# ZhuoyangLiu2005/MLA

Measured on AMD Instinct MI355X. Metric: training samples/sec + step-time, MLA-Llama2-7B bf16, higher is better.
Workload: dtype bf16; 1 GPU; BASELINE.json configs[1]: MLA-Llama2-7B SFT, use_pointcloud+use_contrastive, 672x672(+mask) image + 1024 points + 32 text tokens, per-GPU batch 8 x 4 diffusion repeats = 32 x 548 tokens; model=mla-llama2-7b, global_batch=8, seq_len=548, parallelism=single-gpu, activation_save_level=1, optimizer=fused AdamW + grad clip inside the timed region

## Files before the change

### mla_amd/csrc/gemm256.hip

```cpp
#include "common.h"

#include "gemm_args.h"

#include "gemm256_kloop_clobbers.inc"
#ifndef MLA_GEMM_PLAIN_STORES
#define MLA_ST16(ADDR, VAL) __builtin_nontemporal_store((u32x4_t)(VAL), (u32x4_t*)(ADDR))
#define MLA_LD16(ADDR) __builtin_nontemporal_load((const u32x4_t*)(ADDR))
#else
#define MLA_ST16(ADDR, VAL) (*(u32x4_t*)(ADDR) = (VAL))
#define MLA_LD16(ADDR) (*(const u32x4_t*)(ADDR))
#endif

namespace {

constexpr int SLOT = 16384;
constexpr int SA0 = 0, SB0 = SLOT, SB1 = 2 * SLOT, SA1 = 3 * SLOT, BUF = 4 * SLOT;

__device__ __forceinline__ int hsw(int kr) { return (kr & 3) | (((kr >> 3) & 1) << 2); }
__device__ __forceinline__ int xcd_remap(int bid, int nwg) {
  const int q = nwg >> 3, r = nwg & 7;
  const int xcd = bid & 7, idx = bid >> 3;
  return (xcd < r ? xcd * (q + 1) : r * (q + 1) + (xcd - r) * q) + idx;
}

template <int MODE, bool IS_A>
__device__ __forceinline__ const bf16_t* stage_src(const bf16_t* g, int ld, int base, int lim, int h, int instr, int lane) {
  const int p = instr * 64 + lane;
  if (MODE == 0) {
    const int rp = p >> 3, cp = p & 7;
    const int c = cp ^ (rp & 7);
    int gi = base + h * 128 + rp;
    gi = gi < lim ? gi : lim - 1;
    return g + (size_t)gi * ld + c * 8;
  } else {
    const int kr = p >> 4, cp = p & 15;
    const int c = cp ^ (hsw(kr) << 1);
    const int ip = c * 8;
    int gi = base + h * 128 + ip;
    gi = (gi + 8 <= lim) ? gi : 0;
    return g + (size_t)kr * ld + gi;
  }
}

#ifndef MLA_GROUP_M
#define MLA_GROUP_M 4
#endif
#ifndef MLA_GEMM256_UNTRACKED
#define MLA_GEMM256_UNTRACKED 0
#endif
template <int AMODE, int BMODE, int EPI = 0, bool ASM = false>
__global__ __launch_bounds__(512, 2) void gemm256_kernel(GemmArgs p) {
  const bool LGKM_BEFORE = false;
  const int GROUP_M = MLA_GROUP_M;
#ifdef MLA_GEMM256_ABLATION
  const bool NO_READ = (p.debug & 4) != 0, NO_STAGE = (p.debug & 8) != 0, NO_BAR2 = (p.debug & 16) != 0, NO_BAR1 = (p.debug & 32) != 0;
  const int dbg = p.debug;
#else
  constexpr bool NO_READ = false, NO_STAGE = false, NO_BAR2 = false, NO_BAR1 = false;
  constexpr int dbg = 0;
#endif
  extern __shared__ __attribute__((aligned(16))) char smem[];
  const int tid = threadIdx.x, lane = tid & 63;
  const int wave = __builtin_amdgcn_readfirstlane(tid >> 6);
  const int wr = wave >> 2, wc = wave & 3;
  const int li = lane & 15, lg = lane >> 4;

  const int num_m = (p.M + 255) / 256, num_n = (p.N + 255) / 256;
  int pid, kt0 = 0, nt = p.K / 64;
  float* part = nullptr;
  if (p.sk_split <= 1) {
    pid = xcd_remap(blockIdx.x, gridDim.x);
  } else if ((int)blockIdx.x < p.sk_full) {
    pid = xcd_remap(blockIdx.x, p.sk_full);
  } else {
    const int u = blockIdx.x - p.sk_full;
    const int slice = u % p.sk_split;
    pid = p.sk_full + u / p.sk_split;
    if ((nt & 1) == 0) {
      const int np = nt >> 1;
      kt0 = 2 * (int)((long long)slice * np / p.sk_split);
      nt = 2 * (int)((long long)(slice + 1) * np / p.sk_split) - kt0;
    } else {
    kt0 = (int)((long long)slice * nt / p.sk_split);
    nt = (int)((long long)(slice + 1) * nt / p.sk_split) - kt0;
    }
    part = p.sk_ws + (size_t)u * 65536;
  }
#ifdef MLA_EXPERIMENTAL_KERNELS
  if (EPI != 0 && p.stagger_mode && (int)blockIdx.x < 256) {
    const bool late = p.stagger_mode == 1 ? (blockIdx.x & 1) : ((blockIdx.x >> 3) & 1);
    if (late) {
      const unsigned long long t0 = wall_clock64();
      while ((long long)(wall_clock64() - t0) < (long long)p.stagger_ticks) __builtin_amdgcn_s_sleep(64);
    }
  }
#endif
  const int in_group = GROUP_M * num_n;
  const int group_id = pid / in_group;
  const int first_m = group_id * GROUP_M;
  const int gsz = (num_m - first_m) < GROUP_M ? (num_m - first_m) : GROUP_M;
  const int pid_m = first_m + (pid % in_group) % gsz;
  const int pid_n = (pid % in_group) / gsz;
  const int m0 = pid_m * 256, n0 = pid_n * 256;

  f32x4_t acc[8][4];
  if constexpr (ASM) {
    static_assert(AMODE == 0 && BMODE == 0, "the assembly loop takes k-contiguous operands");
    const unsigned c0 = ((unsigned)lg ^ ((unsigned)li & 7u)) << 4;
    const unsigned vA0 = (unsigned)((wr * 64 + li) * 128) + c0, vB0 = 32768u + (unsigned)((wc * 32 + li) * 128) + c0;
    const unsigned lchunk = ((unsigned)lane & 7u) ^ (((unsigned)lane >> 3) & 7u);
    const int rt0 = wave * 32 + (lane >> 3);
    const int lastA = (p.M - 1 - m0) < 255 ? (p.M - 1 - m0) : 255;
    int lastB = (p.N - 1 - n0) < 255 ? (p.N - 1 - n0) : 255, bshift = 0;
    const bf16_t* pB = p.B + (size_t)n0 * p.ldb + (size_t)kt0 * 64;
    if (EPI == 1) {
      pB = p.B + (size_t)pid_n * 128 * p.ldb;
      bshift = wave >= 4 ? p.sf_I - 128 : 0;
      lastB = 255;
    }
    const unsigned oA0 = (unsigned)rt0 * (unsigned)p.lda * 2u + lchunk * 16u;
    const unsigned oB0 = (unsigned)(rt0 + bshift) * (unsigned)p.ldb * 2u + lchunk * 16u;
    const unsigned oAmax = (unsigned)lastA * (unsigned)p.lda * 2u + lchunk * 16u;
    const unsigned oBmax = (unsigned)(lastB + bshift) * (unsigned)p.ldb * 2u + lchunk * 16u;
    const int sA8 = p.lda * 16, sB8 = p.ldb * 16;
    const bf16_t* pA = p.A + (size_t)m0 * p.lda + (size_t)kt0 * 64;
    const int kmax = nt * 128 - 128, nit = nt >> 1, ldsw = wave * 4096;
    const bool img_bf16 = !part && !p.out_fp32 && p.R == nullptr && p.bias == nullptr;
    const bool rowscale = img_bf16 && p.rs_rstd != nullptr;
    if (rowscale && tid < 256) {
      const int mr = (m0 + tid) < p.M ? (m0 + tid) : (p.M - 1);
      float r;
      if (p.rs_ss) {
        const float* sp = p.rs_ss + (size_t)mr * p.rs_parts;
        float t = 0.f;
        for (int j = 0; j < p.rs_parts; ++j) t += sp[j];
        r = 1.0f / sqrtf(t / (float)p.K + p.rs_eps);
        if (pid_n == 0 && m0 + tid < p.M) p.rs_rstd[mr] = r;
      } else {
        r = p.rs_rstd[mr];
      }
      *(float*)(smem + 2 * BUF + tid * 4) = r;
    }
    const int emode = img_bf16 ? (rowscale ? 2 : 0) : 1;
    const float alpha = part ? 1.f : p.alpha;
    const unsigned vImg = img_bf16 ? (unsigned)((wr * 64 + li) * 512) + ((((unsigned)(wc * 4 + (lg >> 1))) ^ (unsigned)li) << 4) + (unsigned)(lg & 1) * 8u
                                   : (unsigned)((wr * 64 + li) * 1024) + ((((unsigned)(wc * 8 + lg)) ^ (unsigned)li) << 4);
#if defined(__HIP_DEVICE_COMPILE__)
    asm volatile(
#include "gemm256_kloop.inc"
        : : [pA] "s"(pA), [pB] "s"(pB), [kmax] "v"(kmax), [nit] "v"(nit), [ldsw] "s"(ldsw), [sA8] "s"(sA8), [sB8] "s"(sB8),
            [emode] "v"(emode), [alpha] "v"(alpha), [vA0] "v"(vA0), [vB0] "v"(vB0), [oA0] "v"(oA0), [oB0] "v"(oB0), [oAmax] "v"(oAmax),
            [oBmax] "v"(oBmax), [vImg] "v"(vImg)
        : "memory", "scc", "vcc", "s40", "s41", "s42", "s43", "s44", "s45", "s46", "s47", "s48", "s49", "s50", "s51", "s52", "s53", G256K_CLOBBERS);
#endif
    if constexpr (EPI == 0) if (part) {
#pragma unroll
      for (int hf = 0; hf < 2; ++hf) {
        if (hf) {
          __syncthreads();
#if defined(__HIP_DEVICE_COMPILE__)
          asm volatile(
#include "gemm256_kloop_half1.inc"
              : : [alpha] "v"(alpha), [vImg] "v"(vImg) : "memory", "v0", "v1", "v2", "v3", "v4", "v5", "v6", "v7", "v8", "v9", "v10", "v11",
                "v12", "v13", "v14", "v15", "v16", "v17", "v18", "v19");
#endif
        }
        __syncthreads();
#pragma unroll
        for (int it = 0; it < 16; ++it) {
          const int row = wave * 16 + it;
          *(f32x4_t*)(part + (hf * 128 + row) * 256 + lane * 4) = *(const f32x4_t*)(smem + row * 1024 + ((lane ^ (row & 63)) << 4));
        }
      }
      return;
    }
  } else {
  const size_t stepA = (dbg & 64) ? 0 : (dbg & 2) ? 64 : (AMODE == 0 ? 64 : (size_t)64 * p.lda);
  const size_t stepB = (dbg & 64) ? 0 : (dbg & 2) ? 64 : (BMODE == 0 ? 64 : (size_t)64 * p.ldb);
  const bf16_t* pA0[2]; const bf16_t* pA1[2]; const bf16_t* pB0[2]; const bf16_t* pB1[2];
#pragma unroll
  for (int it = 0; it < 2; ++it) {
    if (dbg & 2) {
      pA0[it] = stage_src<0, true>(p.A, 4096, 0, 4096, 0, wave * 2 + it, lane);
      pA1[it] = stage_src<0, true>(p.A, 4096, 0, 4096, 1, wave * 2 + it, lane);
      pB0[it] = stage_src<0, false>(p.B, 4096, 0, 4096, 0, wave * 2 + it, lane);
      pB1[it] = stage_src<0, false>(p.B, 4096, 0, 4096, 1, wave * 2 + it, lane);
      continue;
    }
    pA0[it] = stage_src<AMODE, true>(p.A, p.lda, m0, p.M, 0, wave * 2 + it, lane);
    pA1[it] = stage_src<AMODE, true>(p.A, p.lda, m0, p.M, 1, wave * 2 + it, lane);
    if (EPI == 1) {
      pB0[it] = stage_src<BMODE, false>(p.B, p.ldb, pid_n * 128, p.sf_I, 0, wave * 2 + it, lane);
      pB1[it] = stage_src<BMODE, false>(p.B, p.ldb, p.sf_I + pid_n * 128 - 128, 2 * p.sf_I, 1, wave * 2 + it, lane);
      continue;
    }
    pB0[it] = stage_src<BMODE, false>(p.B, p.ldb, n0, p.N, 0, wave * 2 + it, lane);
    pB1[it] = stage_src<BMODE, false>(p.B, p.ldb, n0, p.N, 1, wave * 2 + it, lane);
  }
  if (kt0) {
#pragma unroll
    for (int it = 0; it < 2; ++it) {
      pA0[it] += (size_t)kt0 * stepA; pA1[it] += (size_t)kt0 * stepA;
      pB0[it] += (size_t)kt0 * stepB; pB1[it] += (size_t)kt0 * stepB;
    }
  }
  int tA0 = 0, tA1 = 0, tB0 = 0, tB1 = 0;
  constexpr bool UNTRACKED = (AMODE != 0 || BMODE != 0) || MLA_GEMM256_UNTRACKED;

#define STAGE(PTR, TCNT, STEP, SLOTOFF)                                                           \
  do {                                                                                            \
    const size_t back__ = (TCNT < nt) ? 0 : (size_t)TCNT * (STEP);  \
    char* dst__ = smem + (TCNT & 1) * BUF + (SLOTOFF) + wave * 2048;                              \
    if (!NO_STAGE || TCNT < 2) {  \
      if (UNTRACKED) {                                                                            \
        glds16_untracked(PTR[0] - back__, dst__);                                                 \
        glds16_untracked(PTR[1] - back__, dst__ + 1024);                                          \
      } else {                                                                                    \
        glds16(PTR[0] - back__, dst__);                                                           \
        glds16(PTR[1] - back__, dst__ + 1024);                                                    \
      }                                                                                           \
    }                                                                                             \
    PTR[0] += (STEP); PTR[1] += (STEP); ++TCNT;                                                   \
  } while (0)

  int offA[4], offB[2];
  if (AMODE == 0) {
    offA[0] = (wr * 64 + li) * 128 + ((lg ^ (li & 7)) * 16);
    offA[1] = offA[2] = offA[3] = 0;
  } else {
    const int h = ((li >> 2) & 3) | ((lg & 1) << 2);
#pragma unroll
    for (int rb = 0; rb < 4; ++rb)
      offA[rb] = ((lg * 8 + (li >> 2)) * 16 + ((wr * 8 + rb * 2 + ((li & 3) >> 1)) ^ (h << 1))) * 16 + (li & 1) * 8;
  }
  if (BMODE == 0) {
    offB[0] = (wc * 32 + li) * 128 + ((lg ^ (li & 7)) * 16);
    offB[1] = 0;
  } else {
    const int h = ((li >> 2) & 3) | ((lg & 1) << 2);
#pragma unroll
    for (int cb = 0; cb < 2; ++cb)
      offB[cb] = ((lg * 8 + (li >> 2)) * 16 + ((wc * 4 + cb * 2 + ((li & 3) >> 1)) ^ (h << 1))) * 16 + (li & 1) * 8;
  }

  auto ldA = [&](const char* slot, int rb, int ks) -> bf16x8_t {
    if (AMODE == 0) {
      return *(const bf16x8_t*)(slot + ((offA[0] + rb * 2048) ^ (ks * 64)));
    } else {
      if (dbg & 1) return *(const bf16x8_t*)(slot + (((wr * 64 + li) * 128 + ((lg ^ (li & 7)) * 16) + rb * 2048) ^ (ks * 64)));
      union { bf16x8_t v; short4_t h2[2]; } u;
      u.h2[0] = lds_tr16_b64(slot + offA[rb] + ks * 8192);
      u.h2[1] = lds_tr16_b64(slot + offA[rb] + ks * 8192 + 1024);
      return u.v;
    }
  };
  auto ldB = [&](const char* slot, int cb, int ks) -> bf16x8_t {
    if (BMODE == 0) {
      return *(const bf16x8_t*)(slot + ((offB[0] + cb * 2048) ^ (ks * 64)));
    } else {
      if (dbg & 1) return *(const bf16x8_t*)(slot + (((wc * 32 + li) * 128 + ((lg ^ (li & 7)) * 16) + cb * 2048) ^ (ks * 64)));
      union { bf16x8_t v; short4_t h2[2]; } u;
      u.h2[0] = lds_tr16_b64(slot + offB[cb] + ks * 8192);
      u.h2[1] = lds_tr16_b64(slot + offB[cb] + ks * 8192 + 1024);
      return u.v;
    }
  };

#pragma unroll
  for (int a = 0; a < 8; ++a)
#pragma unroll
    for (int b = 0; b < 4; ++b) acc[a][b] = f32x4_t{0.f, 0.f, 0.f, 0.f};

  bf16x8_t fa[4][2], fb0[2][2], fb1[2][2];
  bool rd_on = true;

#define READ_A(SLOTP)                                              \
  if (rd_on) _Pragma("unroll") for (int rb = 0; rb < 4; ++rb) {    \
    fa[rb][0] = ldA(SLOTP, rb, 0); fa[rb][1] = ldA(SLOTP, rb, 1);  \
  }
#define READ_B(DST, SLOTP)                                          \
  if (rd_on) _Pragma("unroll") for (int cb = 0; cb < 2; ++cb) {     \
    DST[cb][0] = ldB(SLOTP, cb, 0); DST[cb][1] = ldB(SLOTP, cb, 1); \
  }
#define SEG_END()                                                  \
  __builtin_amdgcn_sched_barrier(0);                               \
  if (LGKM_BEFORE) asm volatile("s_waitcnt vmcnt(8) lgkmcnt(0)" ::: "memory"); \
  else asm volatile("s_waitcnt vmcnt(10)" ::: "memory");           \
  if (!NO_BAR1) __builtin_amdgcn_s_barrier();                      \
  asm volatile("s_waitcnt lgkmcnt(0)" ::: "memory");               \
  __builtin_amdgcn_sched_barrier(0);
#define MMA(QI, QJ, FB)                                                                                          \
  __builtin_amdgcn_s_setprio(1);                                                                                 \
  _Pragma("unroll") for (int ks = 0; ks < 2; ++ks)                                                               \
  _Pragma("unroll") for (int rb = 0; rb < 4; ++rb)                                                               \
  _Pragma("unroll") for (int cb = 0; cb < 2; ++cb)                                                               \
    acc[QI * 4 + rb][QJ * 2 + cb] =                                                                              \
        __builtin_amdgcn_mfma_f32_16x16x32_bf16(FB[cb][ks], fa[rb][ks], acc[QI * 4 + rb][QJ * 2 + cb], 0, 0, 0); \
  __builtin_amdgcn_s_setprio(0);                                                                                 \
  __builtin_amdgcn_sched_barrier(0);                                                                             \
  asm volatile("" ::: "memory");                                                                                 \
  if (!NO_BAR2) __builtin_amdgcn_s_barrier();                                                                    \
  asm volatile("" ::: "memory");

  STAGE(pB0, tB0, stepB, SB0);
  STAGE(pA0, tA0, stepA, SA0);
  STAGE(pB1, tB1, stepB, SB1);
  STAGE(pA1, tA1, stepA, SA1);
  STAGE(pB0, tB0, stepB, SB0);
  STAGE(pA0, tA0, stepA, SA0);
  STAGE(pB1, tB1, stepB, SB1);
  asm volatile("s_waitcnt vmcnt(10)" ::: "memory");
  __builtin_amdgcn_s_barrier();
  READ_B(fb0, smem + SB0)
  if (wr == 1) __builtin_amdgcn_s_barrier();

#define TILE_BODY(X, Y, T_)                                          \
  {                                                                  \
    const char* buf = smem + ((T_) & 1) * BUF;                       \
    const char* nbuf = smem + (((T_) + 1) & 1) * BUF;                \
    if (NO_READ) rd_on = (T_) < 2;                                   \
    STAGE(pA1, tA1, stepA, SA1);                       \
    READ_A(buf + SA0)                                                \
    SEG_END()                                                        \
    MMA(0, 0, X)                                                     \
    STAGE(pB0, tB0, stepB, SB0);                       \
    READ_B(Y, buf + SB1)                                             \
    SEG_END()                                                        \
    MMA(0, 1, Y)                                                     \
    STAGE(pA0, tA0, stepA, SA0);                       \
    READ_A(buf + SA1)                                                \
    SEG_END()                                                        \
    MMA(1, 1, Y)                                                     \
    STAGE(pB1, tB1, stepB, SB1);                       \
    READ_B(Y, nbuf + SB0)                                            \
    SEG_END()                                                        \
    MMA(1, 0, X)                                                     \
  }
  int t = 0;
  for (; t + 1 < nt; t += 2) {
    TILE_BODY(fb0, fb1, t)
    TILE_BODY(fb1, fb0, t + 1)
  }
  if (t < nt) TILE_BODY(fb0, fb1, t)
#undef TILE_BODY
  if (wr == 0) __builtin_amdgcn_s_barrier();
  asm volatile("s_waitcnt vmcnt(0)" ::: "memory");
  }

  if constexpr (!ASM) if (part) {
#pragma unroll
    for (int ri = 0; ri < 8; ++ri) {
      const int ml = (ri >> 2) * 128 + wr * 64 + (ri & 3) * 16 + li;
#pragma unroll
      for (int ci = 0; ci < 4; ++ci) {
        const int nl = (ci >> 1) * 128 + wc * 32 + (ci & 1) * 16 + lg * 4;
        *(f32x4_t*)(part + ml * 256 + nl) = acc[ri][ci];
      }
    }
    return;
  }
  const bool vec_ok = ((p.ldc & 3) == 0) && (p.R == nullptr || (p.ldr & 3) == 0);
  const bool fast = (p.N & 7) == 0 && (p.ldc & 7) == 0 && (((uintptr_t)p.C) & 15) == 0 &&
                    (p.R == nullptr || ((p.ldr & 7) == 0 && (((uintptr_t)p.R) & 15) == 0)) &&
                    (p.bias == nullptr || (((uintptr_t)p.bias) & 15) == 0);
  if (fast) {
    __syncthreads();
    if (!p.out_fp32 && p.R == nullptr && p.bias == nullptr) {
      if constexpr (!ASM) {
      if (p.rs_rstd) {
        if (tid < 256) {
          const int mr = (m0 + tid) < p.M ? (m0 + tid) : (p.M - 1);
          float r;
          if (p.rs_ss) {
            const float* sp = p.rs_ss + (size_t)mr * p.rs_parts;
            float t = 0.f;
            for (int j = 0; j < p.rs_parts; ++j) t += sp[j];
            r = 1.0f / sqrtf(t / (float)p.K + p.rs_eps);
            if (pid_n == 0 && m0 + tid < p.M) p.rs_rstd[mr] = r;
          } else {
            r = p.rs_rstd[mr];
          }
          *(float*)(smem + 2 * BUF + tid * 4) = r;
        }
        __syncthreads();
      }
#pragma unroll
      for (int ri = 0; ri < 8; ++ri) {
        const int ml = (ri >> 2) * 128 + wr * 64 + (ri & 3) * 16 + li;
        const float rsc = p.rs_rstd ? *(const float*)(smem + 2 * BUF + ml * 4) : p.alpha;
#pragma unroll
        for (int ci = 0; ci < 4; ++ci) {
          const int nl = (ci >> 1) * 128 + wc * 32 + (ci & 1) * 16 + lg * 4;
          u32x2_t o;
          o[0] = pack2bf(acc[ri][ci][0] * rsc, acc[ri][ci][1] * rsc);
          o[1] = pack2bf(acc[ri][ci][2] * rsc, acc[ri][ci][3] * rsc);
          *(u32x2_t*)(smem + ml * 512 + ((((nl >> 3) ^ (ml & 31))) << 4) + ((nl >> 2) & 1) * 8) = o;
        }
      }
      }
      __syncthreads();
      if (EPI == 1) {
        const int I = p.sf_I, cbase = pid_n * 128;
        const size_t ld2 = (size_t)2 * I;
        for (int s4 = 0; s4 < 4; ++s4) {
          char* scrA = smem + s4 * 64 * 512;
          u32x4_t pa[2];
#pragma unroll
          for (int k4 = 0; k4 < 4; ++k4) {
            const int idx = tid + 512 * k4;
            const int rl = idx >> 5, ch = idx & 31;
            const int row = s4 * 64 + rl, m = m0 + row;
            if (p.C && m < p.M)
              MLA_ST16((bf16_t*)p.C + (size_t)m * ld2 + (ch < 16 ? cbase + ch * 8 : I + cbase + (ch - 16) * 8), *(const u32x4_t*)(smem + row * 512 + ((ch ^ (row & 31)) << 4)));
          }
#pragma unroll
          for (int k2 = 0; k2 < 2; ++k2) {
            const int idx = tid + 512 * k2;
            const int rl = idx >> 4, c = idx & 15;
            const int row = s4 * 64 + rl, m = m0 + row;
            float gv[8], uv[8], o[8];
            unpack8(*(const u32x4_t*)(smem + row * 512 + ((c ^ (row & 31)) << 4)), gv);
            unpack8(*(const u32x4_t*)(smem + row * 512 + (((16 + c) ^ (row & 31)) << 4)), uv);
#pragma unroll
            for (int j = 0; j < 8; ++j) o[j] = swiglu_fwd_elem(gv[j], uv[j]);
            pa[k2] = pack8(o);
            if (p.sf_act && m < p.M) MLA_ST16(p.sf_act + (size_t)m * I + cbase + c * 8, pa[k2]);
          }
          if (p.sf_actT == nullptr) continue;
          __syncthreads();
#pragma unroll
          for (int k2 = 0; k2 < 2; ++k2) {
            const int idx = tid + 512 * k2;
            const int rl = idx >> 4, c = idx & 15;
            const int slot2 = (rl ^ (2 * c)) * 2;
#pragma unroll
            for (int j = 0; j < 4; ++j) {
              const int c0 = (c * 8 + 2 * j) * 128 + slot2;
              *(unsigned short*)(scrA + c0) = (unsigned short)(pa[k2][j] & 0xffffu);
              *(unsigned short*)(scrA + c0 + 128) = (unsigned short)(pa[k2][j] >> 16);
            }
          }
          __syncthreads();
#pragma unroll
          for (int k2 = 0; k2 < 2; ++k2) {
            const int idx = tid + 512 * k2;
            const int col = idx >> 3, rc = idx & 7;
            const int chc = col >> 3, b = chc & 3;
            const int m = m0 + s4 * 64 + rc * 8;
            if (m < p.M) {
              u32x4_t w = *(const u32x4_t*)(scrA + col * 128 + ((rc ^ (chc >> 2)) << 4));
              if (b & 1) w = u32x4_t{w[1], w[0], w[3], w[2]};
              if (b & 2) w = u32x4_t{w[2], w[3], w[0], w[1]};
              MLA_ST16(p.sf_actT + (size_t)(cbase + col) * p.sf_ldt + m, w);
            }
          }
        }
        return;
      }
      if (EPI == 2) {
        const int I = p.sw_I;
        char* scrB = smem + 2 * BUF;
        const size_t ld2 = (size_t)2 * I;
        u32x4_t gq[4], uq[4];
        auto fetch_gu = [&](int strip, u32x4_t* g4, u32x4_t* u4) {
#pragma unroll
          for (int k4 = 0; k4 < 4; ++k4) {
            const int idx = tid + 512 * k4;
            const int m = m0 + strip * 64 + (idx >> 5), n = n0 + (idx & 31) * 8;
            g4[k4] = u32x4_t{0u, 0u, 0u, 0u};
            u4[k4] = g4[k4];
            if (m < p.M && n < p.N) {
              g4[k4] = MLA_LD16(p.sw_gu + (size_t)m * ld2 + n);
              u4[k4] = MLA_LD16(p.sw_gu + (size_t)m * ld2 + I + n);
            }
          }
        };
        if constexpr (ASM) fetch_gu(0, gq, uq);
        for (int s4 = 0; s4 < 4; ++s4) {
          char* scrA = smem + s4 * 64 * 512;
          u32x4_t pg[4], pu[4];
          u32x4_t gn[4], un[4];
          if constexpr (ASM) if (s4 < 3) fetch_gu(s4 + 1, gn, un);
#pragma unroll
          for (int k4 = 0; k4 < 4; ++k4) {
            const int idx = tid + 512 * k4;
            const int rl = idx >> 5, ch = idx & 31;
            const int row = s4 * 64 + rl;
            const int m = m0 + row, n = n0 + ch * 8;
            pg[k4] = u32x4_t{0u, 0u, 0u, 0u};
            pu[k4] = pg[k4];
            if (m < p.M && n < p.N) {
              float dv[8], gv[8], uv[8], dg[8], du[8];
              unpack8(*(const u32x4_t*)(smem + row * 512 + ((ch ^ (row & 31)) << 4)), dv);
              if constexpr (ASM) {
                unpack8(gq[k4], gv);
                unpack8(uq[k4], uv);
              } else {
              unpack8(*(const u32x4_t*)(p.sw_gu + (size_t)m * ld2 + n), gv);
              unpack8(*(const u32x4_t*)(p.sw_gu + (size_t)m * ld2 + I + n), uv);
              }
#pragma unroll
              for (int j = 0; j < 8; ++j) swiglu_bwd_elem(dv[j], gv[j], uv[j], dg[j], du[j]);
              pg[k4] = pack8(dg);
              pu[k4] = pack8(du);
              MLA_ST16(p.sw_dgu + (size_t)m * ld2 + n, pg[k4]);
              MLA_ST16(p.sw_dgu + (size_t)m * ld2 + I + n, pu[k4]);
            }
          }
          __syncthreads();
#pragma unroll
          for (int k4 = 0; k4 < 4; ++k4) {
            const int idx = tid + 512 * k4;
            const int rl = idx >> 5, ch = idx & 31;
            const int slot2 = (rl ^ (2 * ch)) * 2;
#pragma unroll
            for (int j = 0; j < 4; ++j) {
              const int c0 = (ch * 8 + 2 * j) * 128 + slot2;
              *(unsigned short*)(scrA + c0) = (unsigned short)(pg[k4][j] & 0xffffu);
              *(unsigned short*)(scrA + c0 + 128) = (unsigned short)(pg[k4][j] >> 16);
              *(unsigned short*)(scrB + c0) = (unsigned short)(pu[k4][j] & 0xffffu);
              *(unsigned short*)(scrB + c0 + 128) = (unsigned short)(pu[k4][j] >> 16);
            }
          }
          __syncthreads();
#pragma unroll
          for (int k4 = 0; k4 < 4; ++k4) {
            const int idx = tid + 512 * k4;
            const int col = idx >> 3, rc = idx & 7;
            const int chc = col >> 3;
            const int off = col * 128 + ((rc ^ (chc >> 2)) << 4);
            const int b = chc & 3;
            const int m = m0 + s4 * 64 + rc * 8, n = n0 + col;
            if (m < p.M && n < p.N) {
#pragma unroll
              for (int which = 0; which < 2; ++which) {
                u32x4_t w = *(const u32x4_t*)((which ? scrB : scrA) + off);
                if (b & 1) w = u32x4_t{w[1], w[0], w[3], w[2]};
                if (b & 2) w = u32x4_t{w[2], w[3], w[0], w[1]};
                MLA_ST16(p.sw_dguT + (size_t)(which * I + n) * p.sw_ldt + m, w);
              }
            }
          }
          if constexpr (ASM) {
#pragma unroll
            for (int k4 = 0; k4 < 4; ++k4) { gq[k4] = gn[k4]; uq[k4] = un[k4]; }
          }
        }
        return;
      }
      const int ch = lane & 31;
      const int n = n0 + ch * 8;
      if (p.rope_cos && n0 < p.rope_cols) {
        if (n < p.N) {
          const bool lo = (ch & 8) == 0;
#pragma unroll 4
          for (int it = 0; it < 16; ++it) {
            const int row = wave * 32 + it * 2 + (lane >> 5);
            const int m = m0 + row;
            if (m < p.M) {
              float own[8], par[8], c[8], sn[8], o[8];
              unpack8(*(const u32x4_t*)(smem + row * 512 + ((ch ^ (row & 31)) << 4)), own);
              unpack8(*(const u32x4_t*)(smem + row * 512 + (((ch ^ 8) ^ (row & 31)) << 4)), par);
              const float* ct = p.rope_cos + (size_t)(m % p.rope_S) * 64 + (ch & 7) * 8;
              const float* st = p.rope_sin + (size_t)(m % p.rope_S) * 64 + (ch & 7) * 8;
              const f32x4_t c0 = *(const f32x4_t*)ct, c1 = *(const f32x4_t*)(ct + 4), s0 = *(const f32x4_t*)st, s1 = *(const f32x4_t*)(st + 4);
#pragma unroll
              for (int j = 0; j < 4; ++j) { c[j] = c0[j]; c[j + 4] = c1[j]; sn[j] = s0[j]; sn[j + 4] = s1[j]; }
#pragma unroll
              for (int j = 0; j < 8; ++j)
                o[j] = lo ? fmaf(own[j], c[j], -(par[j] * sn[j])) : fmaf(own[j], c[j], par[j] * sn[j]);
              MLA_ST16((bf16_t*)p.C + (size_t)m * p.ldc + n, pack8(o));
            }
          }
        }
        return;
      }
      if (n < p.N) {
#pragma unroll
        for (int it = 0; it < 16; ++it) {
          const int row = wave * 32 + it * 2 + (lane >> 5);
          const int m = m0 + row;
          if (m < p.M)
            MLA_ST16((bf16_t*)p.C + (size_t)m * p.ldc + n, *(const u32x4_t*)(smem + row * 512 + ((ch ^ (row & 31)) << 4)));
        }
      }
      return;
    }
    if constexpr (EPI == 0 || !ASM) {
    float sq = 0.f;
    u32x4_t rpre[2][8];
    const bool r_pre = ASM && p.R != nullptr && !p.out_fp32;
    if (r_pre) {
      const int nn = n0 + (lane & 31) * 8;
#pragma unroll
      for (int h2 = 0; h2 < 2; ++h2)
#pragma unroll
        for (int it = 0; it < 8; ++it) {
          const int m = m0 + h2 * 128 + wave * 16 + it * 2 + (lane >> 5);
          rpre[h2][it] = u32x4_t{0u, 0u, 0u, 0u};
          if (m < p.M && nn < p.N) rpre[h2][it] = MLA_LD16(p.R + (size_t)m * p.ldr + nn);
        }
    }
#pragma unroll
    for (int hf = 0; hf < 2; ++hf) {
      if (hf) __syncthreads();
      if constexpr (ASM) {
#if defined(__HIP_DEVICE_COMPILE__)
        if (hf) {
          const unsigned vImg2 = (unsigned)((wr * 64 + li) * 1024) + ((((unsigned)(wc * 8 + lg)) ^ (unsigned)li) << 4);
          asm volatile(
#include "gemm256_kloop_half1.inc"
              : : [alpha] "v"(p.alpha), [vImg] "v"(vImg2) : "memory", "v0", "v1", "v2", "v3", "v4", "v5", "v6", "v7", "v8", "v9", "v10",
                "v11", "v12", "v13", "v14", "v15", "v16", "v17", "v18", "v19");
        }
#endif
      } else {
#pragma unroll
      for (int r4 = 0; r4 < 4; ++r4) {
        const int ri = hf * 4 + r4;
        const int ml = wr * 64 + r4 * 16 + li;
#pragma unroll
        for (int ci = 0; ci < 4; ++ci) {
          const int nl = (ci >> 1) * 128 + wc * 32 + (ci & 1) * 16 + lg * 4;
          *(f32x4_t*)(smem + ml * 1024 + (((nl >> 2) ^ (ml & 63)) << 4)) = acc[ri][ci] * p.alpha;
        }
      }
      }
      __syncthreads();
      if (p.out_fp32) {
        const int n = n0 + lane * 4;
        if (n < p.N) {
#pragma unroll
          for (int it = 0; it < 16; ++it) {
            const int row = wave * 16 + it;
            const int m = m0 + hf * 128 + row;
            if (m < p.M) {
              f32x4_t o = *(const f32x4_t*)(smem + row * 1024 + ((lane ^ (row & 63)) << 4));
              if (p.bias) {
                const u32x2_t bb = *(const u32x2_t*)(p.bias + n);
                o[0] += bflo(bb[0]); o[1] += bfhi(bb[0]); o[2] += bflo(bb[1]); o[3] += bfhi(bb[1]);
              }
              if (p.R) {
                const u32x2_t rr = *(const u32x2_t*)(p.R + (size_t)m * p.ldr + n);
                o[0] += bflo(rr[0]); o[1] += bfhi(rr[0]); o[2] += bflo(rr[1]); o[3] += bfhi(rr[1]);
              }
              float* c = (float*)p.C + (size_t)m * p.ldc + n;
              if (p.accumulate) o += *(const f32x4_t*)c;
              *(f32x4_t*)c = o;
              sq += (o[0] * o[0] + o[1] * o[1]) + (o[2] * o[2] + o[3] * o[3]);
            }
          }
        }
      } else {
        const int ch = lane & 31;
        const int n = n0 + ch * 8;
        if (n < p.N) {
          float bv[8];
#pragma unroll
          for (int j = 0; j < 8; ++j) bv[j] = 0.f;
          if (p.bias) unpack8(*(const u32x4_t*)(p.bias + n), bv);
          float ngv[8];
#pragma unroll
          for (int j = 0; j < 8; ++j) ngv[j] = 0.f;
          if (p.nrm_xg) unpack8(*(const u32x4_t*)(p.nrm_g + n), ngv);
#pragma unroll
          for (int it = 0; it < 8; ++it) {
            const int row = wave * 16 + it * 2 + (lane >> 5);
            const int m = m0 + hf * 128 + row;
            if (m < p.M) {
              const f32x4_t a = *(const f32x4_t*)(smem + row * 1024 + (((2 * ch) ^ (row & 63)) << 4));
              const f32x4_t b = *(const f32x4_t*)(smem + row * 1024 + (((2 * ch + 1) ^ (row & 63)) << 4));
              float v[8] = {a[0] + bv[0], a[1] + bv[1], a[2] + bv[2], a[3] + bv[3], b[0] + bv[4], b[1] + bv[5], b[2] + bv[6], b[3] + bv[7]};
              if (p.R) {
                float rv[8];
                unpack8(r_pre ? rpre[hf][it] : *(const u32x4_t*)(p.R + (size_t)m * p.ldr + n), rv);
#pragma unroll
                for (int j = 0; j < 8; ++j) v[j] += rv[j];
              }
              const u32x4_t hq = pack8(v);
              MLA_ST16((bf16_t*)p.C + (size_t)m * p.ldc + n, hq);
              if (p.nrm_xg) {
                float hv[8], xg[8];
                unpack8(hq, hv);
                float q = 0.f;
#pragma unroll
                for (int j = 0; j < 8; ++j) { q += hv[j] * hv[j]; xg[j] = hv[j] * ngv[j]; }
                MLA_ST16(p.nrm_xg + (size_t)m * p.ldc + n, pack8(xg));
                q = half_wave_sum_last(q);
                if (ch == 31) p.nrm_ss[(size_t)m * num_n + pid_n] = q;
              }
            }
          }
        }
      }
    }
    if (p.sq_out) {
      sq = wave_sum(sq);
      __syncthreads();
      if (lane == 0) ((float*)smem)[wave] = sq;
      __syncthreads();
      if (tid == 0) {
        float t = 0.f;
#pragma unroll
        for (int w = 0; w < 8; ++w) t += ((float*)smem)[w];
        p.sq_out[pid] = t;
      }
    }
    }
    return;
  }
  if constexpr (!ASM) {
#pragma unroll
  for (int ri = 0; ri < 8; ++ri) {
    const int m = m0 + (ri >> 2) * 128 + wr * 64 + (ri & 3) * 16 + li;
    if (m >= p.M) continue;

#pragma unroll
    for (int ci = 0; ci < 4; ++ci) {
      const int n = n0 + (ci >> 1) * 128 + wc * 32 + (ci & 1) * 16 + lg * 4;
      if (n >= p.N) continue;
      float v[4];
#pragma unroll
      for (int r = 0; r < 4; ++r) v[r] = acc[ri][ci][r] * p.alpha;
      if (n + 3 < p.N && vec_ok) {
        if (p.bias) {
          const u32x2_t bb = *(const u32x2_t*)(p.bias + n);
          v[0] += bflo(bb[0]); v[1] += bfhi(bb[0]); v[2] += bflo(bb[1]); v[3] += bfhi(bb[1]);
        }
        if (p.R) {
          const u32x2_t rr = *(const u32x2_t*)(p.R + (size_t)m * p.ldr + n);
          v[0] += bflo(rr[0]); v[1] += bfhi(rr[0]); v[2] += bflo(rr[1]); v[3] += bfhi(rr[1]);
        }
        if (p.out_fp32) {
          float* c = (float*)p.C + (size_t)m * p.ldc + n;
          f32x4_t o = {v[0], v[1], v[2], v[3]};
          if (p.accumulate) o += *(const f32x4_t*)c;
          *(f32x4_t*)c = o;
        } else {
          u32x2_t o;
          o[0] = pack2bf(v[0], v[1]);
          o[1] = pack2bf(v[2], v[3]);
          *(u32x2_t*)((bf16_t*)p.C + (size_t)m * p.ldc + n) = o;
        }
      } else {
        for (int r = 0; r < 4 && n + r < p.N; ++r) {
          float x = v[r];
          if (p.bias) x += bf2f(p.bias[n + r]);
          if (p.R) x += bf2f(p.R[(size_t)m * p.ldr + n + r]);
          if (p.out_fp32) {
            float* c = (float*)p.C + (size_t)m * p.ldc + n + r;
            *c = p.accumulate ? (*c + x) : x;
          } else {
            ((bf16_t*)p.C)[(size_t)m * p.ldc + n + r] = f2bf(x);
          }
        }
      }
    }
  }
  }
#undef STAGE
#undef READ_A
#undef READ_B
#undef SEG_END
#undef MMA
}

#ifdef MLA_EXPERIMENTAL_KERNELS
struct Unit {
  int m0, n0, kt0, nt;
  float* part;
};

__global__ __launch_bounds__(512, 2) void gemm256p_kernel(GemmArgs p) {
  const int GROUP_M = MLA_GROUP_M;
  extern __shared__ __attribute__((aligned(16))) char smem[];
  const int tid = threadIdx.x, lane = tid & 63;
  const int wave = __builtin_amdgcn_readfirstlane(tid >> 6);
  const int wr = wave >> 2, wc = wave & 3;
  const int li = lane & 15, lg = lane >> 4;
  const int num_m = (p.M + 255) / 256, num_n = (p.N + 255) / 256;
  const int ntK = p.K / 64;

  const int G = gridDim.x, W = G >> 3, b = blockIdx.x, x = b & 7, j = b >> 3;
  const int F = p.sk_split > 1 ? p.sk_full : num_m * num_n;
  const int q8 = F >> 3, r8 = F & 7;
  const int cnt_x = q8 + (x < r8 ? 1 : 0);
  const int start_x = x < r8 ? x * (q8 + 1) : r8 * (q8 + 1) + (x - r8) * q8;
  const int nfull = j < cnt_x ? (cnt_x - j + W - 1) / W : 0;
  const int tail_units = p.sk_split > 1 ? (num_m * num_n - p.sk_full) * p.sk_split : 0;
  const int ntail = b < tail_units ? (tail_units - b + G - 1) / G : 0;
  const int n_units = nfull + ntail;
  if (n_units == 0) return;
  auto get_unit = [&](int i) -> Unit {
    Unit u;
    int pid;
    if (i < nfull) {
      pid = start_x + j + W * i;
      u.kt0 = 0; u.nt = ntK; u.part = nullptr;
    } else {
      const int t = b + (i - nfull) * G;
      const int slice = t % p.sk_split;
      pid = p.sk_full + t / p.sk_split;
      u.kt0 = (int)((long long)slice * ntK / p.sk_split);
      u.nt = (int)((long long)(slice + 1) * ntK / p.sk_split) - u.kt0;
      u.part = p.sk_ws + (size_t)t * 65536;
    }
    const int in_group = GROUP_M * num_n;
    const int first_m = (pid / in_group) * GROUP_M;
    const int gsz = (num_m - first_m) < GROUP_M ? (num_m - first_m) : GROUP_M;
    u.m0 = __builtin_amdgcn_readfirstlane((first_m + (pid % in_group) % gsz) * 256);
    u.n0 = __builtin_amdgcn_readfirstlane(((pid % in_group) / gsz) * 256);
    u.kt0 = __builtin_amdgcn_readfirstlane(u.kt0);
    u.nt = __builtin_amdgcn_readfirstlane(u.nt);
    return u;
  };

  const int rowA = p.lda * 2, rowB = p.ldb * 2;
  const char* gbA0; const char* gbA1; const char* gbB0; const char* gbB1;
  unsigned voA0[2], voA1[2], voB0[2], voB1[2];
  int stA0 = 128, stA1 = 128, stB0 = 128, stB1 = 128;
  int leftA0, leftB0, leftB1, leftA1, suA0 = 0, suB0 = 0, suB1 = 0, suA1 = 0, tA0 = 0, tB0 = 0, tB1 = 0, tA1 = 0;
#define PSLOT_SET(X, U, ISA, HALF)                                                                                  \
  do {                                                                                                              \
    const int lim_rows__ = (ISA) ? p.M : p.N;                                                                       \
    int hb__ = ((ISA) ? (U).m0 : (U).n0) + (HALF) * 128;                                                            \
    int lim__ = lim_rows__ - 1 - hb__;                                                                              \
    if (lim__ < 0) { hb__ = lim_rows__ - 128; lim__ = 127; }       \
    lim__ = lim__ < 127 ? lim__ : 127;                                                                              \
    gb##X = (const char*)((ISA) ? p.A : p.B) + (size_t)hb__ * ((ISA) ? rowA : rowB) + (size_t)(U).kt0 * 128;        \
    _Pragma("unroll") for (int it__ = 0; it__ < 2; ++it__) {                                                        \
      const int q__ = (wave * 2 + it__) * 64 + lane;                                                                \
      const int rp__ = q__ >> 3, cp__ = q__ & 7;                                                                    \
      const int c__ = cp__ ^ (rp__ & 7);                                                                            \
      const int re__ = rp__ < lim__ ? rp__ : lim__;                                                                 \
      vo##X[it__] = (unsigned)((re__ * ((ISA) ? p.lda : p.ldb) + c__ * 8) * 2);                                     \
    }                                                                                                               \
    left##X = (U).nt;                                                                                               \
  } while (0)
  Unit cu = get_unit(0);
  PSLOT_SET(A0, cu, true, 0);
  PSLOT_SET(A1, cu, true, 1);
  PSLOT_SET(B0, cu, false, 0);
  PSLOT_SET(B1, cu, false, 1);

#define PSTAGE(X, ISA, HALF, SLOTOFF)                                                                                      \
  do {                                                                                                                     \
    char* dst__ = smem + (t##X & 1) * BUF + (SLOTOFF) + wave * 2048;                                                       \
    glds16(gb##X + vo##X[0], dst__);                                                                                       \
    glds16(gb##X + vo##X[1], dst__ + 1024);                                                                                \
    gb##X += st##X; ++t##X;                                                                                                \
// ... 597 lines not shown
```

Before: 14.14 samples/s.

## Restructure SwiGLU GEMM epilogues into per-wave tiles with wave-local transpose

```diff
diff --git a/mla_amd/csrc/gemm256.hip b/mla_amd/csrc/gemm256.hip
--- a/mla_amd/csrc/gemm256.hip
+++ b/mla_amd/csrc/gemm256.hip
@@ -1,6 +1,8 @@
 #include "common.h"
 
 #include "gemm_args.h"
+
+#include <type_traits>
 
 #include "gemm256_kloop_clobbers.inc"
 #ifndef MLA_GEMM_PLAIN_STORES
@@ -39,6 +41,37 @@
     int gi = base + h * 128 + ip;
     gi = (gi + 8 <= lim) ? gi : 0;
     return g + (size_t)kr * ld + gi;
+  }
+}
+
+__device__ __forceinline__ void wave_transpose_store(char* smem, int r0, int G, const u32x4_t (&pk)[8], int lane, bf16_t* outT,
+                                                     long long ldt, int m_left, int n_left) {
+  const int c8 = lane & 7, rq = ((lane >> 3) & 3) * 2 + (lane >> 5);
+  char* const wl = smem + (r0 + c8 * 8) * 512 + ((G ^ (c8 & 3)) << 7);
+  asm volatile("" ::: "memory");
+#pragma unroll
+  for (int i = 0; i < 8; ++i) {
+    const int sb = ((i * 8 + rq) ^ (8 * c8)) * 2;
+#pragma unroll
+    for (int j = 0; j < 4; ++j) {
+      *(unsigned short*)(wl + (2 * j) * 512 + sb) = (unsigned short)(pk[i][j] & 0xffffu);
+      *(unsigned short*)(wl + (2 * j + 1) * 512 + sb) = (unsigned short)(pk[i][j] >> 16);
+    }
+  }
+  asm volatile("" ::: "memory");
+  const int rc = lane & 7, l8 = lane >> 3;
+  u32x4_t w[8];
+#pragma unroll
+  for (int i = 0; i < 8; ++i) {
+    const int cc = (l8 >> 1) | ((i & 1) << 2) | ((l8 & 1) << 3) | ((i >> 1) << 4);
+    const int cw = cc >> 3;
+    w[i] = *(const u32x4_t*)(smem + (r0 + cc) * 512 + ((G ^ (cw & 3)) << 7) + ((rc ^ cw) << 4));
+  }
+  asm volatile("" ::: "memory");
+#pragma unroll
+  for (int i = 0; i < 8; ++i) {
+    const int cc = (l8 >> 1) | ((i & 1) << 2) | ((l8 & 1) << 3) | ((i >> 1) << 4);
+    if (rc * 8 < m_left && cc < n_left) MLA_ST16(outT + (size_t)cc * ldt + rc * 8, w[i]);
   }
 }
 
@@ -399,153 +432,96 @@
       }
       }
       __syncthreads();
+      const int es = wave >> 1, eh = wave & 1, er0 = es * 64;
+      const int c8 = lane & 7, rq = ((lane >> 3) & 3) * 2 + (lane >> 5);
       if (EPI == 1) {
-        const int I = p.sf_I, cbase = pid_n * 128;
+        if (m0 + er0 >= p.M) return;
+        const int I = p.sf_I, cbase = pid_n * 128 + eh * 64;
         const size_t ld2 = (size_t)2 * I;
-        for (int s4 = 0; s4 < 4; ++s4) {
-          char* scrA = smem + s4 * 64 * 512;
-          u32x4_t pa[2];
-#pragma unroll
-          for (int k4 = 0; k4 < 4; ++k4) {
-            const int idx = tid + 512 * k4;
-            const int rl = idx >> 5, ch = idx & 31;
-            const int row = s4 * 64 + rl, m = m0 + row;
-            if (p.C && m < p.M)
-              MLA_ST16((bf16_t*)p.C + (size_t)m * ld2 + (ch < 16 ? cbase + ch * 8 : I + cbase + (ch - 16) * 8), *(const u32x4_t*)(smem + row * 512 + ((ch ^ (row & 31)) << 4)));
+        u32x4_t pa[8];
+#pragma unroll
+        for (int i = 0; i < 8; ++i) {
+          const int row = er0 + i * 8 + rq, m = m0 + row;
+          const u32x4_t gc = *(const u32x4_t*)(smem + row * 512 + (((eh * 8 + c8) ^ (row & 31)) << 4));
+          const u32x4_t uc = *(const u32x4_t*)(smem + row * 512 + (((16 + eh * 8 + c8) ^ (row & 31)) << 4));
+          if (p.C && m < p.M) {
+            MLA_ST16((bf16_t*)p.C + (size_t)m * ld2 + cbase + c8 * 8, gc);
+            MLA_ST16((bf16_t*)p.C + (size_t)m * ld2 + I + cbase + c8 * 8, uc);
           }
-#pragma unroll
-          for (int k2 = 0; k2 < 2; ++k2) {
-            const int idx = tid + 512 * k2;
-            const int rl = idx >> 4, c = idx & 15;
-            const int row = s4 * 64 + rl, m = m0 + row;
-            float gv[8], uv[8], o[8];
-            unpack8(*(const u32x4_t*)(smem + row * 512 + ((c ^ (row & 31)) << 4)), gv);
-            unpack8(*(const u32x4_t*)(smem + row * 512 + (((16 + c) ^ (row & 31)) << 4)), uv);
-#pragma unroll
-            for (int j = 0; j < 8; ++j) o[j] = swiglu_fwd_elem(gv[j], uv[j]);
-            pa[k2] = pack8(o);
-            if (p.sf_act && m < p.M) MLA_ST16(p.sf_act + (size_t)m * I + cbase + c * 8, pa[k2]);
-          }
-          if (p.sf_actT == nullptr) continue;
-          __syncthreads();
-#pragma unroll
-          for (int k2 = 0; k2 < 2; ++k2) {
-            const int idx = tid + 512 * k2;
-            const int rl = idx >> 4, c = idx & 15;
-            const int slot2 = (rl ^ (2 * c)) * 2;
-#pragma unroll
-            for (int j = 0; j < 4; ++j) {
-              const int c0 = (c * 8 + 2 * j) * 128 + slot2;
-              *(unsigned short*)(scrA + c0) = (unsigned short)(pa[k2][j] & 0xffffu);
-              *(unsigned short*)(scrA + c0 + 128) = (unsigned short)(pa[k2][j] >> 16);
+          float gv[8], uv[8], o[8];
+          unpack8(gc, gv);
+          unpack8(uc, uv);
+#pragma unroll
+          for (int j = 0; j < 8; ++j) o[j] = swiglu_fwd_elem(gv[j], uv[j]);
+          pa[i] = pack8(o);
+          if (p.sf_act && m < p.M) MLA_ST16(p.sf_act + (size_t)m * I + cbase + c8 * 8, pa[i]);
+        }
+        if (p.sf_actT == nullptr) return;
+        wave_transpose_store(smem, er0, eh, pa, lane, p.sf_actT + (size_t)cbase * p.sf_ldt + m0 + er0, p.sf_ldt, p.M - m0 - er0, 64);
+        return;
+      }
+      if (EPI == 2) {
+        const int nw = n0 + eh * 128;
+        if (m0 + er0 >= p.M || nw >= p.N) return;
+        const int I = p.sw_I;
+        const size_t ld2 = (size_t)2 * I;
+        auto bwd_wave = [&](auto full_c) {
+          constexpr bool FULL = decltype(full_c)::value;
+          auto fetch_gu = [&](int pass, u32x4_t* g8, u32x4_t* u8) {
+#pragma unroll
+            for (int i = 0; i < 8; ++i) {
+              const int m = m0 + er0 + i * 8 + rq, n = nw + pass * 64 + c8 * 8;
+              g8[i] = u32x4_t{0u, 0u, 0u, 0u};
+              u8[i] = g8[i];
+              if (FULL || (m < p.M && n < p.N)) {
+                g8[i] = MLA_LD16(p.sw_gu + (size_t)m * ld2 + n);
+                u8[i] = MLA_LD16(p.sw_gu + (size_t)m * ld2 + I + n);
+              }
             }
-          }
-          __syncthreads();
-#pragma unroll
-          for (int k2 = 0; k2 < 2; ++k2) {
-            const int idx = tid + 512 * k2;
-            const int col = idx >> 3, rc = idx & 7;
-            const int chc = col >> 3, b = chc & 3;
-            const int m = m0 + s4 * 64 + rc * 8;
-            if (m < p.M) {
-              u32x4_t w = *(const u32x4_t*)(scrA + col * 128 + ((rc ^ (chc >> 2)) << 4));
-              if (b & 1) w = u32x4_t{w[1], w[0], w[3], w[2]};
-              if (b & 2) w = u32x4_t{w[2], w[3], w[0], w[1]};
-              MLA_ST16(p.sf_actT + (size_t)(cbase + col) * p.sf_ldt + m, w);
+        };
+          u32x4_t gq[8], uq[8];
+          fetch_gu(0, gq, uq);
+#pragma unroll
+          for (int ps = 0; ps < 2; ++ps) {
+            const int np = nw + ps * 64;
+            if (!FULL && np >= p.N) break;
+            u32x4_t gn[8], un[8];
+            u32x4_t pg[8], pu[8];
+#pragma unroll
+            for (int i = 0; i < 8; ++i) {
+              const int row = er0 + i * 8 + rq;
+              const int m = m0 + row, n = np + c8 * 8;
+              pg[i] = u32x4_t{0u, 0u, 0u, 0u};
+              pu[i] = pg[i];
+              if (FULL || (m < p.M && n < p.N)) {
+                float dv[8], gv[8], uv[8], dg[8], du[8];
+                unpack8(*(const u32x4_t*)(smem + row * 512 + ((((eh * 2 + ps) * 8 + c8) ^ (row & 31)) << 4)), dv);
+                unpack8(gq[i], gv);
+                unpack8(uq[i], uv);
+#pragma unroll
+                for (int j = 0; j < 8; ++j) swiglu_bwd_elem(dv[j], gv[j], uv[j], dg[j], du[j]);
+                pg[i] = pack8(dg);
+                pu[i] = pack8(du);
+                MLA_ST16(p.sw_dgu + (size_t)m * ld2 + n, pg[i]);
+                MLA_ST16(p.sw_dgu + (size_t)m * ld2 + I + n, pu[i]);
+              }
+              __builtin_amdgcn_sched_barrier(0);
             }
-          }
-        }
-        return;
-      }
-      if (EPI == 2) {
-        const int I = p.sw_I;
-        char* scrB = smem + 2 * BUF;
-        const size_t ld2 = (size_t)2 * I;
-        u32x4_t gq[4], uq[4];
-        auto fetch_gu = [&](int strip, u32x4_t* g4, u32x4_t* u4) {
-#pragma unroll
-          for (int k4 = 0; k4 < 4; ++k4) {
-            const int idx = tid + 512 * k4;
-            const int m = m0 + strip * 64 + (idx >> 5), n = n0 + (idx & 31) * 8;
-            g4[k4] = u32x4_t{0u, 0u, 0u, 0u};
-            u4[k4] = g4[k4];
-            if (m < p.M && n < p.N) {
-              g4[k4] = MLA_LD16(p.sw_gu + (size_t)m * ld2 + n);
-              u4[k4] = MLA_LD16(p.sw_gu + (size_t)m * ld2 + I + n);
+            __builtin_amdgcn_sched_barrier(0);
+            if (ps == 0) fetch_gu(1, gn, un);
+            __builtin_amdgcn_sched_barrier(0);
+            bf16_t* const tT = p.sw_dguT + (size_t)np * p.sw_ldt + m0 + er0;
+            const int ml = FULL ? 64 : p.M - m0 - er0, nl = FULL ? 64 : p.N - np;
+            wave_transpose_store(smem, er0, eh * 2 + ps, pg, lane, tT, p.sw_ldt, ml, nl);
+            wave_transpose_store(smem, er0, eh * 2 + ps, pu, lane, tT + (size_t)I * p.sw_ldt, p.sw_ldt, ml, nl);
+            if (ps == 0) {
+#pragma unroll
+              for (int i = 0; i < 8; ++i) { gq[i] = gn[i]; uq[i] = un[i]; }
             }
           }
         };
-        if constexpr (ASM) fetch_gu(0, gq, uq);
-        for (int s4 = 0; s4 < 4; ++s4) {
-          char* scrA = smem + s4 * 64 * 512;
-          u32x4_t pg[4], pu[4];
-          u32x4_t gn[4], un[4];
-          if constexpr (ASM) if (s4 < 3) fetch_gu(s4 + 1, gn, un);
-#pragma unroll
-          for (int k4 = 0; k4 < 4; ++k4) {
-            const int idx = tid + 512 * k4;
-            const int rl = idx >> 5, ch = idx & 31;
-            const int row = s4 * 64 + rl;
-            const int m = m0 + row, n = n0 + ch * 8;
-            pg[k4] = u32x4_t{0u, 0u, 0u, 0u};
-            pu[k4] = pg[k4];
-            if (m < p.M && n < p.N) {
-              float dv[8], gv[8], uv[8], dg[8], du[8];
-              unpack8(*(const u32x4_t*)(smem + row * 512 + ((ch ^ (row & 31)) << 4)), dv);
-              if constexpr (ASM) {
-                unpack8(gq[k4], gv);
-                unpack8(uq[k4], uv);
-              } else {
-              unpack8(*(const u32x4_t*)(p.sw_gu + (size_t)m * ld2 + n), gv);
-              unpack8(*(const u32x4_t*)(p.sw_gu + (size_t)m * ld2 + I + n), uv);
-              }
-#pragma unroll
-              for (int j = 0; j < 8; ++j) swiglu_bwd_elem(dv[j], gv[j], uv[j], dg[j], du[j]);
-              pg[k4] = pack8(dg);
-              pu[k4] = pack8(du);
-              MLA_ST16(p.sw_dgu + (size_t)m * ld2 + n, pg[k4]);
-              MLA_ST16(p.sw_dgu + (size_t)m * ld2 + I + n, pu[k4]);
-            }
-          }
-          __syncthreads();
-#pragma unroll
-          for (int k4 = 0; k4 < 4; ++k4) {
-            const int idx = tid + 512 * k4;
-            const int rl = idx >> 5, ch = idx & 31;
-            const int slot2 = (rl ^ (2 * ch)) * 2;
-#pragma unroll
-            for (int j = 0; j < 4; ++j) {
-              const int c0 = (ch * 8 + 2 * j) * 128 + slot2;
-              *(unsigned short*)(scrA + c0) = (unsigned short)(pg[k4][j] & 0xffffu);
-              *(unsigned short*)(scrA + c0 + 128) = (unsigned short)(pg[k4][j] >> 16);
-              *(unsigned short*)(scrB + c0) = (unsigned short)(pu[k4][j] & 0xffffu);
-              *(unsigned short*)(scrB + c0 + 128) = (unsigned short)(pu[k4][j] >> 16);
-            }
-          }
-          __syncthreads();
-#pragma unroll
-          for (int k4 = 0; k4 < 4; ++k4) {
-            const int idx = tid + 512 * k4;
-            const int col = idx >> 3, rc = idx & 7;
-            const int chc = col >> 3;
-            const int off = col * 128 + ((rc ^ (chc >> 2)) << 4);
-            const int b = chc & 3;
-            const int m = m0 + s4 * 64 + rc * 8, n = n0 + col;
-            if (m < p.M && n < p.N) {
-#pragma unroll
-              for (int which = 0; which < 2; ++which) {
-                u32x4_t w = *(const u32x4_t*)((which ? scrB : scrA) + off);
-                if (b & 1) w = u32x4_t{w[1], w[0], w[3], w[2]};
-                if (b & 2) w = u32x4_t{w[2], w[3], w[0], w[1]};
-                MLA_ST16(p.sw_dguT + (size_t)(which * I + n) * p.sw_ldt + m, w);
-              }
-            }
-          }
-          if constexpr (ASM) {
-#pragma unroll
-            for (int k4 = 0; k4 < 4; ++k4) { gq[k4] = gn[k4]; uq[k4] = un[k4]; }
-          }
-        }
+        if (ASM && m0 + er0 + 64 <= p.M && nw + 128 <= p.N) bwd_wave(std::integral_constant<bool, ASM>{});
+        else bwd_wave(std::false_type{});
         return;
       }
       const int ch = lane & 31;
```

Result: no change. 14.18 samples/s (median of 6 runs) (+0.3%).
